# moberweger/deep-prior-pp

Hardware: AMD Instinct MI355X
Metric: depth-crops/sec (NYU ResNet50 bs128) 1/2/4/8 GPU; mean 3D joint err (mm) (higher is better)
Workload: dtype f32; 1 GPU; NYU posereg_embedding ResNet (type 0, 30-D PCA prior) train step: fused augment + fwd + bwd + ADAM, bs128/GPU fp32, 128x128x1 crops; global_batch=128, parallelism=dp1, augment=True, augment_pipelined=True, bn=local per-GPU batch statistics, launch_mode=native

## Files before the change

### deep-prior-pp_amd/csrc/stem.hip

```cpp
#include "dpp_common.h"

namespace {

constexpr int KS = 5, PAD = 2, NTAP = 25, KPAD = 28;
constexpr int TC = 16;
constexpr int LX = TC + 2 * PAD;
constexpr int LXP = LX + 1;

template <int CN>
__global__ __launch_bounds__(DPP_THREADS) void stem_fwd_kernel(const float* __restrict__ X, int N, int H, int W, const float* __restrict__ Wk,
                                                               const float* __restrict__ bias, int Co, float* __restrict__ Y,
                                                               uint8_t* __restrict__ arg, int tiles_x, int tiles_y,
                                                               float* __restrict__ stats, int y16) {
    dpp_kernarg_warm<128>();
    __shared__ float xs[LX * LXP];
    __shared__ float Ws[KPAD * CN * 16];
    const int tid = threadIdx.x, wave = tid >> 6, lane = tid & 63, l15 = lane & 15, kq = lane >> 4;
    const int bx = blockIdx.x % tiles_x, by = (blockIdx.x / tiles_x) % tiles_y, n = blockIdx.x / (tiles_x * tiles_y);
    const int cy0 = by * TC, cx0 = bx * TC;
    const int Hp = H >> 1, Wp = W >> 1;
    const float* img = X + (size_t)n * H * W;
    for (int s = tid; s < LX * LX; s += DPP_THREADS) {
        int hy = s / LX, hx = s - hy * LX;
        int y = cy0 + hy - PAD, x = cx0 + hx - PAD;
        xs[hy * LXP + hx] = (y >= 0 && y < H && x >= 0 && x < W) ? img[(size_t)y * W + x] : 0.0f;
    }
    for (int s = tid; s < KPAD * CN * 16; s += DPP_THREADS) {
        int k = s / (CN * 16), o = s - k * (CN * 16);
        Ws[s] = (k < NTAP && o < Co) ? Wk[(size_t)o * NTAP + k] : 0.0f;
    }
    __syncthreads();

    float bf[7][CN];
#pragma unroll
    for (int t = 0; t < 7; ++t)
#pragma unroll
        for (int ct = 0; ct < CN; ++ct) bf[t][ct] = Ws[(4 * t + kq) * (CN * 16) + ct * 16 + l15];
    int koff[7];
    bool kval[7];
#pragma unroll
    for (int t = 0; t < 7; ++t) {
        int k = 4 * t + kq;
        kval[t] = k < NTAP;
        int kk = kval[t] ? k : 0;
        koff[t] = (kk / KS) * LXP + (kk % KS);
    }

    float vals[4][CN];
#pragma unroll
    for (int i = 0; i < 4; ++i)
#pragma unroll
        for (int j = 0; j < CN; ++j) vals[i][j] = 0.0f;
#pragma unroll
    for (int rt = 0; rt < 4; ++rt) {
        const int ply = 2 * wave + (rt >> 1);
        const int qa = l15 >> 2, pa = l15 & 3;
        const int ay = 2 * ply + (pa >> 1), ax = 2 * (((rt & 1) << 2) + qa) + (pa & 1);
        const int abase = ay * LXP + ax;
        f32x4 acc[CN];
#pragma unroll
        for (int ct = 0; ct < CN; ++ct) acc[ct] = (f32x4){0.f, 0.f, 0.f, 0.f};
#pragma unroll
        for (int t = 0; t < 7; ++t) {
            float av = kval[t] ? xs[abase + koff[t]] : 0.0f;
#pragma unroll
            for (int ct = 0; ct < CN; ++ct) acc[ct] = __builtin_amdgcn_mfma_f32_16x16x4f32(av, bf[t][ct], acc[ct], 0, 0, 0);
        }
        const int py = (cy0 >> 1) + ply, px = (cx0 >> 1) + ((rt & 1) << 2) + kq;
        if (py < Hp && px < Wp) {
            size_t o = (((size_t)n * Hp + py) * Wp + px) * Co;
#pragma unroll
            for (int ct = 0; ct < CN; ++ct) {
                int col = ct * 16 + l15;
                if (col < Co) {
                    float best = fmaxf(fmaxf(acc[ct][0], acc[ct][1]), fmaxf(acc[ct][2], acc[ct][3]));
                    int ties = 0;
#pragma unroll
                    for (int r = 0; r < 4; ++r) ties |= (acc[ct][r] == best) ? (1 << r) : 0;
                    if (y16) reinterpret_cast<dpp_bf16*>(Y)[o + col] = (dpp_bf16)(best + bias[col]);
                    else Y[o + col] = best + bias[col];
                    vals[rt][ct] = best + bias[col];
                    if (arg) arg[o + col] = (uint8_t)ties;
                }
            }
        }
    }
    if (stats != nullptr) {
        float sm[CN], m2[CN];
#pragma unroll
        for (int ct = 0; ct < CN; ++ct) sm[ct] = vals[0][ct] + vals[1][ct] + vals[2][ct] + vals[3][ct];
        dpp_tile_colsum<CN, 4, 1, CN * 16>(sm, xs, wave, 0, l15, kq);
#pragma unroll
        for (int ct = 0; ct < CN; ++ct) {
            sm[ct] *= (1.0f / 64.0f);
            float t = 0.0f;
#pragma unroll
            for (int rt = 0; rt < 4; ++rt) { float dv = vals[rt][ct] - sm[ct]; t += dv * dv; }
            m2[ct] = t;
        }
        dpp_tile_colsum<CN, 4, 1, CN * 16>(m2, xs, wave, 0, l15, kq);
        if (kq == 0 && wave == 0) {
#pragma unroll
            for (int ct = 0; ct < CN; ++ct) {
                int col = ct * 16 + l15;
                if (col < Co) {
                    stats[dpp_partial_index(0, col, blockIdx.x, Co, gridDim.x)] = sm[ct];
                    stats[dpp_partial_index(1, col, blockIdx.x, Co, gridDim.x)] = m2[ct];
                }
            }
        }
    }
}

constexpr int LXW = LX + 2;
constexpr int GM_A = 64 * 32 + 16;

__global__ __launch_bounds__(DPP_THREADS) void stem_wgrad_kernel(const float* __restrict__ X, int N, int H, int W, const float* __restrict__ dY,
                                                                 const uint8_t* __restrict__ arg, int Co, float* __restrict__ partial,
                                                                 int tiles_x, int tiles_y, int tiles_per_block, int total_tiles) {
    dpp_kernarg_warm<128>();
    __shared__ __attribute__((aligned(16))) float gm[4 * GM_A];
    __shared__ float xs[LX * LXW];
    const int tid = threadIdx.x, wave = tid >> 6, lane = tid & 63, l15 = lane & 15, kq = lane >> 4;
    const int Hp = H >> 1, Wp = W >> 1;
    const bool vec = (Co & 3) == 0 && (reinterpret_cast<uintptr_t>(dY) & 15) == 0 && (reinterpret_cast<uintptr_t>(arg) & 3) == 0;
    int offB[2];
    bool okB[2];
#pragma unroll
    for (int ct = 0; ct < 2; ++ct) {
        const int tap = ct * 16 + l15;
        okB[ct] = tap < NTAP;
        const int tt = okB[ct] ? tap : 0;
        offB[ct] = ((kq >> 1) + tt / KS) * LXW + (kq & 1) + tt % KS;
    }
    float4 rg[2];
    unsigned rt_[2];
    float rh[2];
    auto load_tile = [&](int tile) {
        const int bx = tile % tiles_x, by = (tile / tiles_x) % tiles_y, n = tile / (tiles_x * tiles_y);
        const int cy0 = by * TC, cx0 = bx * TC;
#pragma unroll
        for (int i = 0; i < 2; ++i) {
            const int item = tid + i * DPP_THREADS, p = item >> 3, oq = item & 7;
            const int py = (cy0 >> 1) + (p >> 3), px = (cx0 >> 1) + (p & 7);
            float4 g = make_float4(0.f, 0.f, 0.f, 0.f);
            unsigned t = 0;
            if (py < Hp && px < Wp && oq * 4 < Co) {
                const size_t idx = (((size_t)n * Hp + py) * Wp + px) * Co + oq * 4;
                if (vec) {
                    g = *reinterpret_cast<const float4*>(dY + idx);
                    t = *reinterpret_cast<const unsigned*>(arg + idx);
                } else {
                    float gv[4] = {0.f, 0.f, 0.f, 0.f};
                    for (int j = 0; j < 4; ++j)
                        if (oq * 4 + j < Co) { gv[j] = dY[idx + j]; t |= (unsigned)arg[idx + j] << (8 * j); }
                    g = make_float4(gv[0], gv[1], gv[2], gv[3]);
                }
            }
            rg[i] = g;
            rt_[i] = t;
        }
        const float* img = X + (size_t)n * H * W;
#pragma unroll
        for (int i = 0; i < 2; ++i) {
            const int s2 = tid + i * DPP_THREADS;
            float v = 0.0f;
            if (s2 < LX * LX) {
                const int hy = s2 / LX, hx = s2 - hy * LX;
                const int y = cy0 + hy - PAD, x = cx0 + hx - PAD;
                if (y >= 0 && y < H && x >= 0 && x < W) v = img[(size_t)y * W + x];
            }
            rh[i] = v;
        }
    };
    auto commit_tile = [&]() {
#pragma unroll
        for (int i = 0; i < 2; ++i) {
            const int item = tid + i * DPP_THREADS, p = item >> 3, oq = item & 7;
            const float4 g = rg[i];
            const unsigned t = rt_[i];
#pragma unroll
            for (int a = 0; a < 4; ++a) {
                float4 m;
                m.x = ((t >> a) & 1u) ? g.x : 0.0f;
                m.y = ((t >> (8 + a)) & 1u) ? g.y : 0.0f;
                m.z = ((t >> (16 + a)) & 1u) ? g.z : 0.0f;
                m.w = ((t >> (24 + a)) & 1u) ? g.w : 0.0f;
                *reinterpret_cast<float4*>(&gm[a * GM_A + p * 32 + oq * 4]) = m;
            }
        }
#pragma unroll
        for (int i = 0; i < 2; ++i) {
            const int s2 = tid + i * DPP_THREADS;
            if (s2 < LX * LX) xs[(s2 / LX) * LXW + s2 % LX] = rh[i];
        }
    };
    f32x4 acc[2][2];
#pragma unroll
    for (int i = 0; i < 2; ++i)
#pragma unroll
        for (int j = 0; j < 2; ++j) acc[i][j] = (f32x4){0.f, 0.f, 0.f, 0.f};
    const int tile0 = blockIdx.x * tiles_per_block;
    int ntiles = total_tiles - tile0;
    if (ntiles > tiles_per_block) ntiles = tiles_per_block;
    if (ntiles > 0) load_tile(tile0);
    for (int ti = 0; ti < ntiles; ++ti) {
        commit_tile();
        __syncthreads();
        if (ti + 1 < ntiles) load_tile(tile0 + ti + 1);
#pragma unroll
        for (int sidx = 0; sidx < 16; ++sidx) {
            const int p = wave * 16 + sidx;
            const int base = (2 * (p >> 3)) * LXW + 2 * (p & 7);
            const float a0 = gm[kq * GM_A + p * 32 + l15], a1 = gm[kq * GM_A + p * 32 + 16 + l15];
            const float b0 = okB[0] ? xs[base + offB[0]] : 0.0f;
            const float b1 = okB[1] ? xs[base + offB[1]] : 0.0f;
            acc[0][0] = __builtin_amdgcn_mfma_f32_16x16x4f32(a0, b0, acc[0][0], 0, 0, 0);
            acc[0][1] = __builtin_amdgcn_mfma_f32_16x16x4f32(a0, b1, acc[0][1], 0, 0, 0);
            acc[1][0] = __builtin_amdgcn_mfma_f32_16x16x4f32(a1, b0, acc[1][0], 0, 0, 0);
            acc[1][1] = __builtin_amdgcn_mfma_f32_16x16x4f32(a1, b1, acc[1][1], 0, 0, 0);
        }
        __syncthreads();
    }
    float* red = gm;
#pragma unroll
    for (int rt = 0; rt < 2; ++rt)
#pragma unroll
        for (int ct = 0; ct < 2; ++ct)
#pragma unroll
            for (int r = 0; r < 4; ++r) red[wave * 1024 + (rt * 16 + kq * 4 + r) * 32 + ct * 16 + l15] = acc[rt][ct][r];
    __syncthreads();
    for (int s2 = tid; s2 < Co * NTAP; s2 += DPP_THREADS) {
        const int oo = s2 / NTAP, k = s2 - oo * NTAP;
        const int at = oo * 32 + k;
        partial[(size_t)blockIdx.x * Co * NTAP + s2] = ((red[at] + red[1024 + at]) + red[2048 + at]) + red[3072 + at];
    }
}

}

extern "C" int dpp_stem_fwd(const float* X, int N, int H, int W, const float* Wk, const float* bias, int Co, float* Y, uint8_t* argmax,
                            float* stats, int store,
                            dpp_stream_t stream) {
    if (!X || !Wk || !bias || !Y || N < 1 || H < 2 || W < 2 || (H & 1) || (W & 1) || Co < 1 || Co > 32 || (store & ~DPP_ST_C)) return DPP_E_BADARG;
    const int y16 = (store & DPP_ST_C) ? 1 : 0;
    if (stats && ((H % TC) || (W % TC))) return DPP_E_BADARG;
    int tiles_x = dpp_cdiv(W, TC), tiles_y = dpp_cdiv(H, TC);
    dim3 grid(tiles_x * tiles_y * N);
    hipStream_t st = static_cast<hipStream_t>(stream);
    if (Co <= 16)
        DPP_LAUNCH((stem_fwd_kernel<1>), grid, dim3(DPP_THREADS), 0, st, X, N, H, W, Wk, bias, Co, Y, argmax, tiles_x, tiles_y, stats, y16);
    else
        DPP_LAUNCH((stem_fwd_kernel<2>), grid, dim3(DPP_THREADS), 0, st, X, N, H, W, Wk, bias, Co, Y, argmax, tiles_x, tiles_y, stats, y16);
    return dpp_launch_status();
}

extern "C" int dpp_stem_wgrad_blocks(int N, int H, int W, int tiles_per_block) {
    int total = dpp_cdiv(W, TC) * dpp_cdiv(H, TC) * N;
    return dpp_cdiv(total, tiles_per_block > 0 ? tiles_per_block : 1);
}

extern "C" int dpp_stem_wgrad(const float* X, int N, int H, int W, const float* dY, const uint8_t* argmax, int Co, float* partial,
                              int tiles_per_block, dpp_stream_t stream) {
    if (!X || !dY || !argmax || !partial || N < 1 || (H & 1) || (W & 1) || Co < 1 || Co > 32 || tiles_per_block < 1)
        return DPP_E_BADARG;
    int tiles_x = dpp_cdiv(W, TC), tiles_y = dpp_cdiv(H, TC);
    int total = tiles_x * tiles_y * N;
    DPP_LAUNCH(stem_wgrad_kernel, dim3(dpp_cdiv(total, tiles_per_block)), dim3(DPP_THREADS), 0, static_cast<hipStream_t>(stream), X, N,
                       H, W, dY, argmax, Co, partial, tiles_x, tiles_y, tiles_per_block, total);
    return dpp_launch_status();
}
```

Baseline: 37930 depth-crops/sec.

## Add persistent MFMA stem forward kernel with double-buffered tile prefetch

Adds a persistent-grid stem forward kernel that walks tiles with a capped grid and prefetches the next input tile into registers, committing it to a double-buffered LDS slot while the current tile computes. The 5x5 convolution runs on 16x16x4 f32 MFMA with weights held in registers, and the 2x2 max-pool and argmax use DPP quad permutes instead of shared memory. Per-tile BN partial statistics are kept. The goal is to cut launch/tile overhead and LDS traffic in the stem conv+pool and to overlap global loads with compute. The cost is much more code complexity, inline asm, and an env-controlled grid size, and the new path only applies to Co of 16 or 32 with aligned pointers.

New measurement: 38050 depth-crops/sec (median of 6 runs). About the same (+0.3%).

```diff
diff --git a/deep-prior-pp_amd/csrc/stem.hip b/deep-prior-pp_amd/csrc/stem.hip
--- a/deep-prior-pp_amd/csrc/stem.hip
+++ b/deep-prior-pp_amd/csrc/stem.hip
@@ -112,6 +112,230 @@
     }
 }
 
+constexpr int WXP = 24;
+
+template <int M, class T>
+__device__ __forceinline__ T quad_xor(T v) {
+    static_assert(sizeof(T) == 4 && (M == 1 || M == 2), "quad_xor");
+#ifdef DPP_HIP_EMU
+    return __shfl_xor(v, M);
+#else
+    int i;
+    __builtin_memcpy(&i, &v, 4);
+    i = __builtin_amdgcn_mov_dpp(i, M == 1 ? 0xB1 : 0x4E, 0xf, 0xf, true);
+    T r;
+    __builtin_memcpy(&r, &i, 4);
+    return r;
+#endif
+}
+
+__device__ __forceinline__ void quad_max4(const f32x4& a, f32x4& m) {
+#ifdef DPP_HIP_EMU
+#pragma unroll
+    for (int r = 0; r < 4; ++r) {
+        float b = fmaxf(a[r], quad_xor<1>(a[r]));
+        m[r] = fmaxf(b, quad_xor<2>(b));
+    }
+#else
+    float m0, m1, m2, m3;
+    asm("s_nop 1\n\t"
+        "v_max_f32_dpp %0, %4, %4 quad_perm:[1,0,3,2] row_mask:0xf bank_mask:0xf\n\t"
+        "v_max_f32_dpp %1, %5, %5 quad_perm:[1,0,3,2] row_mask:0xf bank_mask:0xf\n\t"
+        "v_max_f32_dpp %2, %6, %6 quad_perm:[1,0,3,2] row_mask:0xf bank_mask:0xf\n\t"
+        "v_max_f32_dpp %3, %7, %7 quad_perm:[1,0,3,2] row_mask:0xf bank_mask:0xf\n\t"
+        "v_max_f32_dpp %0, %0, %0 quad_perm:[2,3,0,1] row_mask:0xf bank_mask:0xf\n\t"
+        "v_max_f32_dpp %1, %1, %1 quad_perm:[2,3,0,1] row_mask:0xf bank_mask:0xf\n\t"
+        "v_max_f32_dpp %2, %2, %2 quad_perm:[2,3,0,1] row_mask:0xf bank_mask:0xf\n\t"
+        "v_max_f32_dpp %3, %3, %3 quad_perm:[2,3,0,1] row_mask:0xf bank_mask:0xf"
+        : "=&v"(m0), "=&v"(m1), "=&v"(m2), "=&v"(m3)
+        : "v"(a[0]), "v"(a[1]), "v"(a[2]), "v"(a[3]));
+    m[0] = m0; m[1] = m1; m[2] = m2; m[3] = m3;
+#endif
+}
+
+template <int CN, bool ARG, bool STATS>
+__global__ __launch_bounds__(DPP_THREADS) DPP_WAVES_PER_EU(5, 8) void stem_fwd_walk_kernel(const float* __restrict__ X, int H, int W, const float* __restrict__ Wk,
+                                                                    const float* __restrict__ bias, float* Y,
+                                                                    uint8_t* arg, int tiles_x, int tiles_y, int total_tiles,
+                                                                    float* __restrict__ stats) {
+    constexpr int Co = CN * 16;
+    __shared__ __attribute__((aligned(16))) float xs[2][DPP_THREADS * 4];
+    __shared__ __attribute__((aligned(16))) float sred[2][2][4][Co];
+    const int tid = threadIdx.x, wave = tid >> 6, lane = tid & 63, l15 = lane & 15, kq = lane >> 4;
+    const int q = l15 >> 2, p = l15 & 3;
+    const int Hp = H >> 1, Wp = W >> 1;
+
+    float wf[7][CN];
+#pragma unroll
+    for (int t = 0; t < 7; ++t) {
+        const int k = 4 * t + kq, kc = k < NTAP ? k : NTAP - 1;
+#pragma unroll
+        for (int ct = 0; ct < CN; ++ct) wf[t][ct] = Wk[(ct * 16 + l15) * NTAP + kc];
+    }
+    const int ct_s = CN == 2 ? (p & 1) : 0;
+    const int xh_s = CN == 2 ? (p >> 1) : (p & 1);
+    const int cq = ct_s * 16 + kq * 4;
+    const float4 bq = *reinterpret_cast<const float4*>(bias + cq);
+    const int hs = tid < LX * 6 ? tid : LX * 6 - 1;
+    const int hrow = hs / 6, hc4 = hs - hrow * 6;
+    const int hslot = tid < LX * 6 ? hrow * WXP + hc4 * 4 : tid * 4;
+    float4 hreg;
+    bool hok;
+    auto request = [&](int tile) {
+        const int bx = tile % tiles_x, r2 = tile / tiles_x, by = r2 % tiles_y, n = r2 / tiles_y;
+        const int y = by * TC - PAD + hrow, x = bx * TC - 4 + hc4 * 4;
+        hok = (y >= 0) & (y < H) & (x >= 0) & (x < W);
+        const int yc = y < 0 ? 0 : (y >= H ? H - 1 : y), xc = x < 0 ? 0 : (x >= W ? W - 4 : x);
+        hreg = *reinterpret_cast<const float4*>(X + ((size_t)n * H + yc) * W + xc);
+    };
+    const int G = gridDim.x;
+    int tile = blockIdx.x;
+    request(tile);
+#pragma unroll
+    for (int t = 0; t < 7; ++t)
+#pragma unroll
+        for (int ct = 0; ct < CN; ++ct) wf[t][ct] = (4 * t + kq < NTAP) ? wf[t][ct] : 0.0f;
+    int koff[7];
+#pragma unroll
+    for (int t = 0; t < 7; ++t) {
+        const int k = 4 * t + kq, kk = k < NTAP ? k : 0;
+        koff[t] = (kk / KS) * WXP + (kk % KS) + (4 - PAD);
+    }
+    const int bbase = (4 * wave + (p >> 1)) * WXP + 2 * q + (p & 1);
+
+    auto commit = [&](int buf) {
+        *reinterpret_cast<float4*>(&xs[buf][hslot]) = make_float4(hok ? hreg.x : 0.0f, hok ? hreg.y : 0.0f, hok ? hreg.z : 0.0f, hok ? hreg.w : 0.0f);
+    };
+    int cur = 0;
+    commit(0);
+    for (; tile < total_tiles; tile += G, cur ^= 1) {
+        __syncthreads();
+        const int bx = tile % tiles_x, r2 = tile / tiles_x, by = r2 % tiles_y, n = r2 / tiles_y;
+        {
+            const int nxt = tile + G;
+            request(nxt < total_tiles ? nxt : tile);
+        }
+        DPP_SCHED_FENCE();
+        const float* img = xs[cur];
+        float vs[CN][4];
+        unsigned wsel[CN];
+        size_t off[CN];
+#pragma unroll
+        for (int g = 0; g < CN; ++g) {
+            f32x4 sel = (f32x4){0.f, 0.f, 0.f, 0.f};
+            unsigned ws = 0;
+#pragma unroll
+            for (int c0 = 0; c0 < 4; c0 += CN) {
+                const int rt = CN == 2 ? 2 * g + (c0 >> 1) : c0;
+                const int ab = bbase + (rt >> 1) * 2 * WXP + (rt & 1) * 8;
+                f32x4 acc[CN];
+#pragma unroll
+                for (int ct = 0; ct < CN; ++ct) acc[ct] = (f32x4){0.f, 0.f, 0.f, 0.f};
+#pragma unroll
+                for (int t = 0; t < 7; ++t) {
+                    const float xv = img[ab + koff[t]];
+#pragma unroll
+                    for (int ct = 0; ct < CN; ++ct) acc[ct] = __builtin_amdgcn_mfma_f32_16x16x4f32(wf[t][ct], xv, acc[ct], 0, 0, 0);
+                }
+#pragma unroll
+                for (int ct = 0; ct < CN; ++ct) {
+                    f32x4 m;
+                    unsigned w = 0;
+                    quad_max4(acc[ct], m);
+#pragma unroll
+                    for (int r = 0; r < 4; ++r)
+                        if (ARG) w |= (acc[ct][r] == m[r]) ? (1u << (8 * r)) : 0u;
+                    if (ARG) {
+                        w <<= p;
+                        w |= quad_xor<1>(w);
+                        w |= quad_xor<2>(w);
+                    }
+                    const bool mine = p == c0 + ct;
+#pragma unroll
+                    for (int r = 0; r < 4; ++r) sel[r] = mine ? m[r] : sel[r];
+                    if (ARG) ws = mine ? w : ws;
+                }
+            }
+            const int ply = CN == 2 ? 2 * wave + g : 2 * wave + (p >> 1);
+            const int py = by * (TC / 2) + ply, px = bx * (TC / 2) + xh_s * 4 + q;
+            const size_t o = (((size_t)n * Hp + py) * Wp + px) * Co + cq;
+            const float4 v = make_float4(sel[0] + bq.x, sel[1] + bq.y, sel[2] + bq.z, sel[3] + bq.w);
+            vs[g][0] = v.x; vs[g][1] = v.y; vs[g][2] = v.z; vs[g][3] = v.w;
+            wsel[g] = ws;
+            off[g] = o;
+#ifndef DPP_HIP_EMU
+            asm volatile("" : "+v"(vs[g][0]), "+v"(vs[g][1]), "+v"(vs[g][2]), "+v"(vs[g][3]), "+v"(wsel[g]));
+#endif
+            DPP_SCHED_FENCE();
+        }
+        commit(cur ^ 1);
+        asm volatile("" ::: "memory");
+        DPP_SCHED_FENCE();
+#pragma unroll
+        for (int g = 0; g < CN; ++g) {
+            *reinterpret_cast<float4*>(Y + off[g]) = make_float4(vs[g][0], vs[g][1], vs[g][2], vs[g][3]);
+            if (ARG) *reinterpret_cast<unsigned*>(arg + off[g]) = wsel[g];
+        }
+        if (STATS) {
+            float v4[4][4];
+#pragma unroll
+            for (int j = 0; j < 4; ++j) {
+                if (CN == 2) {
+                    const float x0 = quad_xor<2>(vs[0][j]), x1 = quad_xor<2>(vs[CN - 1][j]);
+                    const bool hi = (p & 2) != 0;
+                    v4[0][j] = hi ? x0 : vs[0][j];
+                    v4[1][j] = hi ? vs[0][j] : x0;
+                    v4[2][j] = hi ? x1 : vs[CN - 1][j];
+                    v4[3][j] = hi ? vs[CN - 1][j] : x1;
+                } else {
+                    const float own = vs[0][j], x1 = quad_xor<1>(own), x2 = quad_xor<2>(own), x3 = quad_xor<2>(x1);
+#pragma unroll
+                    for (int k = 0; k < 4; ++k) {
+                        const int d = p ^ k;
+                        v4[k][j] = d == 0 ? own : (d == 1 ? x1 : (d == 2 ? x2 : x3));
+                    }
+                }
+            }
+            auto tilesum = [&](float (&t)[4], float (*red)[Co]) {
+#pragma unroll
+                for (int j = 0; j < 4; ++j) {
+                    t[j] += __shfl_xor(t[j], 4);
+                    t[j] += __shfl_xor(t[j], 8);
+                }
+                if ((l15 & (CN == 2 ? 14 : 15)) == 0) *reinterpret_cast<float4*>(&red[wave][cq]) = make_float4(t[0], t[1], t[2], t[3]);
+                __syncthreads();
+#pragma unroll
+                for (int j = 0; j < 4; ++j) t[j] = 0.0f;
+#pragma unroll
+                for (int w = 0; w < 4; ++w) {
+                    const float4 r = *reinterpret_cast<const float4*>(&red[w][cq]);
+                    t[0] += r.x; t[1] += r.y; t[2] += r.z; t[3] += r.w;
+                }
+            };
+            float sm[4], m2[4];
+#pragma unroll
+            for (int j = 0; j < 4; ++j) sm[j] = v4[0][j] + v4[1][j] + v4[2][j] + v4[3][j];
+            tilesum(sm, sred[cur][0]);
+#pragma unroll
+            for (int j = 0; j < 4; ++j) {
+                sm[j] *= (1.0f / 64.0f);
+                float t = 0.0f;
+#pragma unroll
+                for (int rt = 0; rt < 4; ++rt) { float dv = v4[rt][j] - sm[j]; t += dv * dv; }
+                m2[j] = t;
+            }
+            tilesum(m2, sred[cur][1]);
+            if (wave == 0 && (l15 & (CN == 2 ? 14 : 15)) == 0) {
+#pragma unroll
+                for (int j = 0; j < 4; ++j) {
+                    stats[dpp_partial_index(0, cq + j, tile, Co, total_tiles)] = sm[j];
+                    stats[dpp_partial_index(1, cq + j, tile, Co, total_tiles)] = m2[j];
+                }
+            }
+        }
+    }
+}
+
 constexpr int LXW = LX + 2;
 constexpr int GM_A = 64 * 32 + 16;
 
@@ -248,6 +472,21 @@
     int tiles_x = dpp_cdiv(W, TC), tiles_y = dpp_cdiv(H, TC);
     dim3 grid(tiles_x * tiles_y * N);
     hipStream_t st = static_cast<hipStream_t>(stream);
+    const char* we = getenv("DPP_STEM_WGS");
+    const int wgs = we ? atoi(we) : 2048;
+    auto al = [](const void* p, uintptr_t a) { return (reinterpret_cast<uintptr_t>(p) & (a - 1)) == 0; };
+    if (wgs > 0 && !y16 && H % TC == 0 && W % TC == 0 && (Co == 16 || Co == 32) && al(X, 16) && al(Y, 16) && al(argmax, 4) && al(bias, 16)) {
+        const int total = (int)grid.x;
+        const dim3 gw(wgs < total ? wgs : total);
+#define DPP_STEM_WALK(CN_, A_, S_) DPP_LAUNCH((stem_fwd_walk_kernel<CN_, A_, S_>), gw, dim3(DPP_THREADS), 0, st, X, H, W, Wk, bias, Y, argmax, tiles_x, tiles_y, total, stats)
+#define DPP_STEM_WALK_AS(CN_) do { \
+            if (argmax) { if (stats) DPP_STEM_WALK(CN_, true, true); else DPP_STEM_WALK(CN_, true, false); } \
+            else { if (stats) DPP_STEM_WALK(CN_, false, true); else DPP_STEM_WALK(CN_, false, false); } } while (0)
+        if (Co == 16) DPP_STEM_WALK_AS(1); else DPP_STEM_WALK_AS(2);
+#undef DPP_STEM_WALK_AS
+#undef DPP_STEM_WALK
+        return dpp_launch_status();
+    }
     if (Co <= 16)
         DPP_LAUNCH((stem_fwd_kernel<1>), grid, dim3(DPP_THREADS), 0, st, X, N, H, W, Wk, bias, Co, Y, argmax, tiles_x, tiles_y, stats, y16);
     else
```
